# DhairyaLGandhi/FluxDistributed.jl

Measured on AMD Instinct MI355X. Metric: images/sec, higher is better.
Workload: dtype bf16; 1 GPU; model=resnet34, global_batch=96, image_size=224, num_classes=1000, parallelism=dp1, engine=graph, optimizer=sgd_momentum(lr=0.01,m=0.9), loss=logitcrossentropy

## Files before the change

fluxdistributed_amd/csrc/bindings.cpp:

```cpp
#include <torch/extension.h>
#include <ATen/hip/HIPContext.h>

#include "fda_kernels.h"

namespace {

using fda::DT;

DT dt_of(const at::Tensor& t) {
    if (t.scalar_type() == at::kBFloat16) return DT::BF16;
    TORCH_CHECK(t.scalar_type() == at::kFloat, "expected f32 or bf16, got ",
                t.scalar_type());
    return DT::F32;
}

hipStream_t cur_stream() {
    return at::hip::getCurrentHIPStream().stream();
}

std::pair<int64_t, int64_t> nhwc_rows(const at::Tensor& x) {
    TORCH_CHECK(x.dim() == 4, "expected 4D NCHW-logical tensor");
    TORCH_CHECK(x.is_contiguous(at::MemoryFormat::ChannelsLast),
                "expected channels_last layout");
    return {x.size(0) * x.size(2) * x.size(3), x.size(1)};
// ... 701 lines not shown
    TORCH_CHECK(w.size(1) == x.size(1), op, ": channel mismatch");
    return g;
}

at::Tensor conv_igemm_fwd(at::Tensor x, at::Tensor w,
                          int64_t sy, int64_t sx, int64_t py, int64_t px) {
    const char* op = "conv_igemm_fwd";
    const auto g = check_fwd(op, x, w, sy, sx, py, px);
    return std::get<0>(conv_run(op, fda::CONV_FWD, x, w, g, false, {}));
}

std::tuple<at::Tensor, at::Tensor> conv_igemm_fwd_stats(
    at::Tensor x, at::Tensor w, int64_t sy, int64_t sx, int64_t py,
    int64_t px) {
    const char* op = "conv_igemm_fwd_stats";
    const auto g = check_fwd(op, x, w, sy, sx, py, px);
    return conv_run(op, fda::CONV_FWD, x, w, g, true, {});
}

at::Tensor conv_igemm_dgrad(at::Tensor dy, at::Tensor wt,
                            int64_t C, int64_t H, int64_t W,
                            int64_t R, int64_t S,
                            int64_t sy, int64_t sx, int64_t py, int64_t px,
                            c10::optional<at::Tensor> accum) {
    const char* op = "conv_igemm_dgrad";
    check_cl_bf16(op, "dy", dy);
    const auto g = conv_geometry(op, dy.size(0), C, H, W, dy.size(1), R, S,
                                 sy, sx, py, px);
    check_dy(op, dy, g);
    TORCH_CHECK(wt.dim() == 2 && wt.scalar_type() == at::kBFloat16 &&
                    wt.is_contiguous() && wt.size(0) == R * S * C &&
                    wt.size(1) == g.K,
                op, ": wt must be contiguous bf16 [R*S*C][K]");
    ConvExtras ex;
    if (accum.has_value() && accum->defined()) {
        ex.accum = *accum;
        TORCH_CHECK(ex.accum.scalar_type() == at::kBFloat16 &&
                        ex.accum.sizes() == at::IntArrayRef({g.N, C, H, W}) &&
                        ex.accum.is_contiguous(at::MemoryFormat::ChannelsLast),
                    op, ": accum must be channels_last bf16 of dx's shape [",
                    g.N, ",", C, ",", H, ",", W, "]");
        check_aligned16(op, "accum", ex.accum);
    }
    return std::get<0>(conv_run(op, fda::CONV_DGRAD, dy, wt, g, false, ex));
}

fda::ConvGeom check_wgrad(const char* op, const at::Tensor& dy,
                          const at::Tensor& x, int64_t R, int64_t S,
                          int64_t sy, int64_t sx, int64_t py, int64_t px) {
    check_cl_bf16(op, "dy", dy);
    check_cl_bf16(op, "x", x);
    const auto g = conv_geometry(op, x.size(0), x.size(1), x.size(2),
                                 x.size(3), dy.size(1), R, S, sy, sx, py, px);
    TORCH_CHECK(dy.size(0) == x.size(0), op, ": batch size mismatch: dy has ",
                dy.size(0), ", x has ", x.size(0));
    check_dy(op, dy, g);
    return g;
}

void conv_igemm_wgrad_into(at::Tensor dy, at::Tensor x, at::Tensor ws,
                           int64_t R, int64_t S,
                           int64_t sy, int64_t sx, int64_t py, int64_t px) {
    const char* op = "conv_igemm_wgrad_into";
    const auto g = check_wgrad(op, dy, x, R, S, sy, sx, py, px);
    check_flat(op, "ws", ws, at::kFloat, (int64_t)g.K * R * S * g.C);
    check_device(op, {dy, x, ws});
    fda::conv_wgrad_launch(dy.data_ptr(), x.data_ptr(), ws.data_ptr<float>(),
                           g, cur_stream());
}

at::Tensor conv_igemm_wgrad(at::Tensor dy, at::Tensor x,
                            int64_t R, int64_t S,
                            int64_t sy, int64_t sx, int64_t py, int64_t px) {
    TORCH_CHECK(dy.dim() == 4 && x.dim() == 4,
                "conv_igemm_wgrad: dy and x must be 4-D");
    auto ws = at::zeros({dy.size(1), R * S * x.size(1)},
                        x.options().dtype(at::kFloat));
    conv_igemm_wgrad_into(dy, x, ws, R, S, sy, sx, py, px);
    return ws;
}

fda::ConvGeom check_stem_geometry(const char* op, const at::Tensor& x8,
                                  int64_t K, int64_t R, int64_t sy, int64_t sx,
                                  int64_t P, int64_t Q) {
    TORCH_CHECK(x8.scalar_type() == at::kBFloat16 && x8.dim() == 4 &&
                    x8.is_contiguous(at::MemoryFormat::ChannelsLast) &&
                    x8.size(1) == 8,
                op, ": x8 must be [N,8,Hp,Wp] channels_last bf16");
    TORCH_CHECK(K >= 64 && K % 64 == 0, op, ": K must be a multiple of 64");
    TORCH_CHECK(R >= 1 && sy >= 1 && sx >= 1 && P >= 1 && Q >= 1 &&
                    (P - 1) * sy + R <= x8.size(2) &&
                    (Q - 1) * sx + 8 <= x8.size(3),
                op, ": output ", P, "x", Q, " reads outside the padded ",
                x8.size(2), "x", x8.size(3), " input");
    fda::ConvGeom g{};
    g.N = (int)x8.size(0); g.H = (int)x8.size(2); g.W = (int)x8.size(3);
    g.C = 8; g.K = (int)K; g.P = (int)P; g.Q = (int)Q; g.R = (int)R; g.S = 1;
    g.sy = (int)sy; g.sx = (int)sx;
    return g;
}

std::tuple<at::Tensor, at::Tensor> conv_stem_run(
    const char* op, const at::Tensor& x8, const at::Tensor& wpad, int64_t R,
    int64_t sy, int64_t sx, int64_t P, int64_t Q, bool want_stats,
    const ConvExtras& ex) {
    TORCH_CHECK(wpad.dim() == 3 && wpad.is_contiguous() &&
                    wpad.scalar_type() == at::kBFloat16 &&
                    wpad.size(1) == R && wpad.size(2) == 64,
                op, ": wpad must be contiguous bf16 [K][R][64]");
    const auto g = check_stem_geometry(op, x8, wpad.size(0), R, sy, sx, P, Q);
    if (ex.scale.defined()) check_epilogue_coeffs(op, ex.scale, ex.shift, g.K);
    check_device(op, {x8, wpad, ex.scale, ex.shift});
    auto y = at::empty({g.N, g.K, g.P, g.Q},
                       x8.options().memory_format(at::MemoryFormat::ChannelsLast));
    at::Tensor part;
    if (want_stats)
        part = at::empty(
            {fda::conv_igemm_plan(g, fda::CONV_STEM).stats_rows, 2, g.K},
            x8.options().dtype(at::kFloat));
    const fda::EpiInfer epi{
        ex.scale.defined() ? ex.scale.data_ptr<float>() : nullptr,
        ex.scale.defined() ? ex.shift.data_ptr<float>() : nullptr, nullptr,
        ex.relu};
    fda::conv_stem_fwd_launch(x8.data_ptr(), wpad.data_ptr(), y.data_ptr(), g,
                              cur_stream(),
                              want_stats ? part.data_ptr<float>() : nullptr,
                              ex.scale.defined() ? &epi : nullptr);
    return {y, part};
}

at::Tensor conv_stem_fwd(at::Tensor x8, at::Tensor wpad, int64_t R,
                         int64_t sy, int64_t sx, int64_t P, int64_t Q) {
    return std::get<0>(conv_stem_run("conv_stem_fwd", x8, wpad, R, sy, sx, P,
                                     Q, false, {}));
}

std::tuple<at::Tensor, at::Tensor> conv_stem_fwd_stats(
    at::Tensor x8, at::Tensor wpad, int64_t R, int64_t sy, int64_t sx,
    int64_t P, int64_t Q) {
    return conv_stem_run("conv_stem_fwd_stats", x8, wpad, R, sy, sx, P, Q,
                         true, {});
}

std::tuple<int64_t, int64_t, int64_t, bool> conv_igemm_fwd_config(
    int64_t M, int64_t C, int64_t K, int64_t R, int64_t S) {
    TORCH_CHECK(M >= 1 && M <= INT32_MAX && C >= 64 && C % 64 == 0 &&
                    K >= 64 && K % 64 == 0 && R >= 1 && S >= 1,
                "conv_igemm_fwd_config: bad geometry");
    fda::ConvGeom g{};
    g.N = 1; g.P = 1; g.Q = (int)M;
    g.C = (int)C; g.K = (int)K; g.R = (int)R; g.S = (int)S;
    const auto plan = fda::conv_igemm_plan(g, fda::CONV_FWD);
    return {plan.bm, plan.bn, plan.sk, plan.ring};
}


at::Tensor conv_igemm_fwd_fused(at::Tensor x, at::Tensor w, at::Tensor scale,
                                at::Tensor shift, at::Tensor residual,
                                bool relu, int64_t sy, int64_t sx, int64_t py,
                                int64_t px) {
    const char* op = "conv_igemm_fwd_fused";
    const auto g = check_fwd(op, x, w, sy, sx, py, px);
    check_epilogue_coeffs(op, scale, shift, g.K);
    ConvExtras ex;
    ex.scale = scale;
    ex.shift = shift;
    ex.relu = relu;
    if (residual.defined() && residual.numel() > 0) {
        TORCH_CHECK(residual.scalar_type() == at::kBFloat16 &&
                        residual.sizes() ==
                            at::IntArrayRef({g.N, g.K, g.P, g.Q}) &&
                        residual.is_contiguous(at::MemoryFormat::ChannelsLast),
                    op, ": residual must be channels_last bf16 of the "
                    "output's shape [", g.N, ",", g.K, ",", g.P, ",", g.Q, "]");
        check_aligned16(op, "residual", residual);
        ex.residual = residual;
    }
    return std::get<0>(conv_run(op, fda::CONV_FWD, x, w, g, false, ex));
}

at::Tensor conv_stem_fwd_fused(at::Tensor x8, at::Tensor wpad,
                               at::Tensor scale, at::Tensor shift, bool relu,
                               int64_t R, int64_t sy, int64_t sx, int64_t P,
                               int64_t Q) {
    ConvExtras ex;
    ex.scale = scale;
    ex.shift = shift;
    ex.relu = relu;
    return std::get<0>(conv_stem_run("conv_stem_fwd_fused", x8, wpad, R, sy,
                                     sx, P, Q, false, ex));
}

void bn_fold_eval_batch(at::Tensor w_ptrs, at::Tensor b_ptrs,
                        at::Tensor rm_ptrs, at::Tensor rv_ptrs, at::Tensor Cs,
                        at::Tensor offs, at::Tensor eps, at::Tensor arena,
                        int64_t max_c) {
    const char* op = "bn_fold_eval_batch";
    const int64_t n = w_ptrs.numel();
    TORCH_CHECK(n >= 1 && n <= 65535, op, ": need 1..65535 layers, got ", n);
    check_flat(op, "w_ptrs", w_ptrs, at::kLong, n);
    check_flat(op, "b_ptrs", b_ptrs, at::kLong, n);
    check_flat(op, "rm_ptrs", rm_ptrs, at::kLong, n);
    check_flat(op, "rv_ptrs", rv_ptrs, at::kLong, n);
    check_flat(op, "Cs", Cs, at::kInt, n);
    check_flat(op, "offs", offs, at::kLong, n);
    check_flat(op, "eps", eps, at::kFloat, n);
    TORCH_CHECK(arena.scalar_type() == at::kFloat && arena.dim() == 1 &&
                    arena.is_contiguous(),
                op, ": arena must be 1-D contiguous fp32");
    TORCH_CHECK(max_c >= 1 && 2 * max_c <= arena.numel(), op,
                ": max_c must be in [1, arena/2], got ", max_c);
    check_device(op, {w_ptrs, b_ptrs, rm_ptrs, rv_ptrs, Cs, offs, eps, arena});
    fda::bn_fold_eval_batch_launch(
        w_ptrs.data_ptr<int64_t>(), b_ptrs.data_ptr<int64_t>(),
        rm_ptrs.data_ptr<int64_t>(), rv_ptrs.data_ptr<int64_t>(),
        Cs.data_ptr<int>(), offs.data_ptr<int64_t>(), eps.data_ptr<float>(),
        arena.data_ptr<float>(), arena.numel(), (int)n, (int)max_c,
        cur_stream());
}

at::Tensor conv_stem_wgrad(at::Tensor dy, at::Tensor x8, int64_t R,
                           int64_t sy, int64_t sx) {
    const char* op = "conv_stem_wgrad";
    TORCH_CHECK(dy.scalar_type() == at::kBFloat16 && dy.dim() == 4 &&
                    dy.is_contiguous(at::MemoryFormat::ChannelsLast),
                op, ": dy must be 4-D channels_last bf16");
    const auto g = check_stem_geometry(op, x8, dy.size(1), R, sy, sx,
                                       dy.size(2), dy.size(3));
    TORCH_CHECK(dy.size(0) == x8.size(0), op, ": batch size mismatch");
    check_device(op, {dy, x8});
    auto ws = at::zeros({g.K, R * 64}, x8.options().dtype(at::kFloat));
    fda::conv_stem_wgrad_launch(dy.data_ptr(), x8.data_ptr(),
                                ws.data_ptr<float>(), g, cur_stream());
    return ws;
}

at::Tensor pad_rows_bf16(at::Tensor src, int64_t ldl) {
    TORCH_CHECK(src.dim() == 2 && src.is_contiguous() &&
                src.scalar_type() == at::kBFloat16);
    const long M = src.size(0);
    const int C = (int)src.size(1);
    TORCH_CHECK(C % 8 == 0 && ldl % 8 == 0 && ldl >= C);
    check_device("pad_rows_bf16", {src});
    auto dst = at::empty({M, ldl}, src.options());
    fda::pad_rows_bf16_launch(dst.data_ptr(), src.data_ptr(), M, C, (int)ldl,
                              cur_stream());
    return dst;
}

void pad_rows_bf16_into(at::Tensor dst, at::Tensor src) {
    TORCH_CHECK(dst.dim() == 2 && src.dim() == 2);
    TORCH_CHECK(dst.is_contiguous() && src.is_contiguous());
    TORCH_CHECK(dst.size(0) == src.size(0));
    TORCH_CHECK(dst.scalar_type() == at::kBFloat16 &&
                    src.scalar_type() == at::kBFloat16,
                "pad_rows_bf16_into: bf16 only");
    TORCH_CHECK(src.size(1) % 8 == 0 && dst.size(1) % 8 == 0 &&
                    src.size(1) <= dst.size(1),
                "pad_rows_bf16_into: row lengths must be multiples of 8 "
                "with src's <= dst's");
    check_device("pad_rows_bf16_into", {dst, src});
    fda::pad_rows_bf16_launch(dst.data_ptr(), src.data_ptr(), src.size(0),
                              (int)src.size(1), (int)dst.size(1),
                              cur_stream());
}

void bias_add_rows_bf16(at::Tensor y, at::Tensor bias) {
    TORCH_CHECK(y.dim() == 2 && y.is_contiguous() &&
                y.scalar_type() == at::kBFloat16);
    TORCH_CHECK(bias.numel() == y.size(1) && bias.is_contiguous() &&
                bias.scalar_type() == at::kBFloat16);
    TORCH_CHECK(y.size(1) % 8 == 0, "bias_add_rows_bf16: row length % 8");
    check_device("bias_add_rows_bf16", {y, bias});
    fda::bias_add_rows_bf16_launch(y.data_ptr(), bias.data_ptr(), y.size(0),
                                   (int)y.size(1), cur_stream());
}

void colsum_accum_bf16(at::Tensor g, at::Tensor dy) {
    TORCH_CHECK(dy.dim() == 2 && dy.is_contiguous() &&
                dy.scalar_type() == at::kBFloat16);
    TORCH_CHECK(g.is_contiguous() && g.scalar_type() == at::kBFloat16);
    TORCH_CHECK(g.numel() <= dy.size(1));
    check_device("colsum_accum_bf16", {g, dy});
    fda::colsum_accum_bf16_launch(g.data_ptr(), dy.data_ptr(), dy.size(0),
                                  (int)dy.size(1), (int)g.numel(),
                                  cur_stream());
}

void grad_accum_batch(at::Tensor g_ptrs, at::Tensor ws_ptrs, at::Tensor ns,
                      int64_t max_n) {
    const int64_t n = g_ptrs.numel();
    check_flat("grad_accum_batch", "g_ptrs", g_ptrs, at::kLong, n);
    check_flat("grad_accum_batch", "ws_ptrs", ws_ptrs, at::kLong, n);
    check_flat("grad_accum_batch", "ns", ns, at::kLong, n);
    check_device("grad_accum_batch", {g_ptrs, ws_ptrs, ns});
    fda::grad_accum_batch_launch(g_ptrs.data_ptr<int64_t>(),
                                 ws_ptrs.data_ptr<int64_t>(),
                                 ns.data_ptr<int64_t>(),
                                 (int)g_ptrs.numel(), max_n, cur_stream());
}

void grad_accum_bf16(at::Tensor g, at::Tensor ws) {
    TORCH_CHECK(g.scalar_type() == at::kBFloat16 && g.is_contiguous());
    TORCH_CHECK(ws.scalar_type() == at::kFloat && ws.is_contiguous());
    TORCH_CHECK(g.numel() == ws.numel());
    check_device("grad_accum_bf16", {g, ws});
// ... 47 lines not shown

at::Tensor preprocess_batch(at::Tensor arena, at::Tensor meta, int64_t crop,
                            bool normalize, bool standardize, bool bf16) {
    TORCH_CHECK(arena.is_cuda() && meta.is_cuda(),
                "preprocess_batch: device tensors required (a CPU tensor here "
                "would fault the GPU with a host pointer)");
    TORCH_CHECK(arena.device() == meta.device(),
                "preprocess_batch: arena and meta must share a device");
    TORCH_CHECK(arena.scalar_type() == at::kByte && arena.dim() == 1 &&
                arena.is_contiguous(),
                "preprocess_batch: arena must be 1-D contiguous uint8");
    TORCH_CHECK(meta.scalar_type() == at::kInt && meta.dim() == 2 &&
                meta.size(1) == fda::PREPROCESS_META_INTS &&
                meta.is_contiguous(),
                "preprocess_batch: meta must be contiguous int32 [N][",
                fda::PREPROCESS_META_INTS, "]");
    TORCH_CHECK((reinterpret_cast<uintptr_t>(arena.data_ptr()) & 15) == 0,
                "preprocess_batch: arena must be 16-byte aligned");
    TORCH_CHECK(crop >= 1 && crop <= 4096,
                "preprocess_batch: crop must be in [1, 4096], got ", crop);
    const int64_t N = meta.size(0);
    const int tiles = fda::preprocess_tiles((int)crop);
    TORCH_CHECK(N * tiles < (int64_t)1 << 31,
                "preprocess_batch: batch too large");
    auto out = at::empty({N, 3, crop, crop},
                         arena.options()
                             .dtype(bf16 ? at::kBFloat16 : at::kFloat)
                             .memory_format(at::MemoryFormat::ChannelsLast));
    if (N == 0) return out;
    auto scratch = at::empty({N, crop, crop, 3},
                             arena.options().dtype(at::kFloat));
    auto partials = at::empty({N, tiles, 2},
                              arena.options().dtype(at::kDouble));
    auto stream = cur_stream();
    fda::preprocess_resample_launch(arena.data_ptr<uint8_t>(), arena.numel(),
                                    meta.data_ptr<int32_t>(),
                                    scratch.data_ptr<float>(),
                                    partials.data_ptr<double>(), (int)N,
                                    (int)crop, normalize, stream);
    fda::preprocess_apply_launch(scratch.data_ptr<float>(),
                                 partials.data_ptr<double>(), out.data_ptr(),
                                 (int)N, (int)crop, standardize,
                                 bf16 ? DT::BF16 : DT::F32, stream);
    return out;
}

}

PYBIND11_MODULE(TORCH_EXTENSION_NAME, m) {
    m.def("preprocess_batch", &preprocess_batch, pybind11::arg("arena"),
          pybind11::arg("meta"), pybind11::arg("crop"),
          pybind11::arg("normalize"), pybind11::arg("standardize"),
          pybind11::arg("bf16"),
          "uint8 image arena -> resized, cropped, normalized NHWC batch");
    m.def("ce_fwd", &ce_fwd, "fused logit cross-entropy fwd (loss + dlogits)");
    m.def("add_relu_fwd", &add_relu_fwd);
    m.def("add_relu_bwd", &add_relu_bwd);
    m.def("bn_act_fwd", &bn_act_fwd, pybind11::arg("x"),
          pybind11::arg("weight"), pybind11::arg("bias"),
          pybind11::arg("running_mean"), pybind11::arg("running_var"),
          pybind11::arg("training"), pybind11::arg("momentum"),
          pybind11::arg("eps"), pybind11::arg("relu"),
          pybind11::arg("residual"),
          pybind11::arg("conv_part") = pybind11::none());
    m.def("bn_act_bwd", &bn_act_bwd, pybind11::arg("gout"),
          pybind11::arg("x"), pybind11::arg("weight"),
          pybind11::arg("save_mean"), pybind11::arg("save_invstd"),
          pybind11::arg("out"), pybind11::arg("relu"),
          pybind11::arg("training"),
          pybind11::arg("gw_out") = pybind11::none(),
          pybind11::arg("gb_out") = pybind11::none(),
          pybind11::arg("want_gres") = false,
          pybind11::arg("bias") = pybind11::none());
    m.def("bn_act_pool_supported", &bn_act_pool_supported);
    m.def("bn_act_pool_fwd", &bn_act_pool_fwd, pybind11::arg("x"),
          pybind11::arg("weight"), pybind11::arg("bias"),
          pybind11::arg("running_mean"), pybind11::arg("running_var"),
          pybind11::arg("training"), pybind11::arg("momentum"),
          pybind11::arg("eps"), pybind11::arg("KH"), pybind11::arg("KW"),
          pybind11::arg("S"), pybind11::arg("P"),
          pybind11::arg("conv_part") = pybind11::none());
    m.def("bn_act_pool_bwd", &bn_act_pool_bwd, pybind11::arg("gout"),
          pybind11::arg("x"), pybind11::arg("weight"), pybind11::arg("bias"),
          pybind11::arg("save_mean"), pybind11::arg("save_invstd"),
          pybind11::arg("idx"), pybind11::arg("KH"), pybind11::arg("KW"),
          pybind11::arg("S"), pybind11::arg("P"), pybind11::arg("training"),
          pybind11::arg("gw_out") = pybind11::none(),
          pybind11::arg("gb_out") = pybind11::none());
    m.def("maxpool_fwd", &maxpool_fwd);
    m.def("maxpool_bwd", &maxpool_bwd);
    m.def("gap_fwd", &gap_fwd);
    m.def("gap_bwd", &gap_bwd);
    m.def("sgd_step", &sgd_step);
    m.def("adam_step", &adam_step);
    m.def("lars_plan", &lars_plan, pybind11::arg("offsets"),
          pybind11::arg("numels"), pybind11::arg("n"),
          pybind11::arg("seg_base"),
          "host chunk table of one flat group: int32 [nchunks][3] rows of "
          "{segment id, start element, own elements}");
    m.def("lars_norms", &lars_norms, pybind11::arg("P"), pybind11::arg("G"),
          pybind11::arg("M"), pybind11::arg("table"),
          pybind11::arg("partials"), pybind11::arg("chunk_base"),
          pybind11::arg("total_chunks"), pybind11::arg("S"));
    m.def("lars_fold", &lars_fold, pybind11::arg("partials"),
          pybind11::arg("seg_meta"), pybind11::arg("lr"),
          pybind11::arg("coef"), pybind11::arg("stats"),
          pybind11::arg("skipped"), pybind11::arg("eta"),
          pybind11::arg("weight_decay"), pybind11::arg("eps"),
          pybind11::arg("max_grad_norm"));
    m.def("lars_step", &lars_step, pybind11::arg("P"), pybind11::arg("G"),
          pybind11::arg("M"), pybind11::arg("V"), pybind11::arg("table"),
          pybind11::arg("seg_meta"), pybind11::arg("coef"),
          pybind11::arg("stats"), pybind11::arg("momentum"),
          pybind11::arg("weight_decay"));
    m.attr("LARS_CHUNK") = fda::LARS_CHUNK;
    m.def("grad_mean_multi", &grad_mean_multi, pybind11::arg("grads"),
          pybind11::arg("flag") = pybind11::none(),
          "in-place mean of R flat gradient buffers (fp32 sum, one round)");
    m.def("conv_igemm_fwd_stats", &conv_igemm_fwd_stats);
    m.def("conv_stem_fwd_stats", &conv_stem_fwd_stats);
    m.def("conv_igemm_fwd", &conv_igemm_fwd,
          "implicit-GEMM conv fwd (NHWC bf16, MFMA)");
    m.def("wt_transpose_batch", &wt_transpose_batch);
    m.def("grad_accum_bf16", &grad_accum_bf16);
    m.def("grad_accum_batch", &grad_accum_batch);
    m.def("pad_rows_bf16", &pad_rows_bf16);
    m.def("pad_rows_bf16_into", &pad_rows_bf16_into);
    m.def("bias_add_rows_bf16", &bias_add_rows_bf16);
    m.def("colsum_accum_bf16", &colsum_accum_bf16);
    m.def("conv_stem_fwd", &conv_stem_fwd);
    m.def("conv_stem_wgrad", &conv_stem_wgrad);
    m.def("conv_igemm_fwd_config", &conv_igemm_fwd_config,
          pybind11::arg("M"), pybind11::arg("C"), pybind11::arg("K"),
          pybind11::arg("R"), pybind11::arg("S"),
          "(BM, BN, SK, ring) of a forward conv with M output pixels");
    m.def("conv_igemm_fwd_fused", &conv_igemm_fwd_fused, pybind11::arg("x"),
          pybind11::arg("w"), pybind11::arg("scale"), pybind11::arg("shift"),
          pybind11::arg("residual"), pybind11::arg("relu"),
          pybind11::arg("sy"), pybind11::arg("sx"), pybind11::arg("py"),
          pybind11::arg("px"),
          "conv + eval BN + residual + ReLU, one bf16 round (inference)");
    m.def("conv_stem_fwd_fused", &conv_stem_fwd_fused, pybind11::arg("x8"),
          pybind11::arg("wpad"), pybind11::arg("scale"),
          pybind11::arg("shift"), pybind11::arg("relu"), pybind11::arg("R"),
          pybind11::arg("sy"), pybind11::arg("sx"), pybind11::arg("P"),
          pybind11::arg("Q"));
    m.def("bn_fold_eval_batch", &bn_fold_eval_batch, pybind11::arg("w_ptrs"),
          pybind11::arg("b_ptrs"), pybind11::arg("rm_ptrs"),
          pybind11::arg("rv_ptrs"), pybind11::arg("Cs"),
          pybind11::arg("offs"), pybind11::arg("eps"), pybind11::arg("arena"),
          pybind11::arg("max_c"),
          "eval-mode BN scale/shift of every layer in one launch");
    m.def("conv_igemm_wgrad_into", &conv_igemm_wgrad_into);
    m.def("conv_igemm_wgrad", &conv_igemm_wgrad,
          "implicit-GEMM conv weight-grad (NHWC bf16, MFMA + tr16 reads)");
    m.def("conv_igemm_dgrad", &conv_igemm_dgrad,
          "implicit-GEMM conv input-grad (NHWC bf16, MFMA; optional fused "
          "+= accum epilogue)",
          pybind11::arg("dy"), pybind11::arg("wt"), pybind11::arg("C"),
          pybind11::arg("H"), pybind11::arg("W"), pybind11::arg("R"),
          pybind11::arg("S"), pybind11::arg("sy"), pybind11::arg("sx"),
          pybind11::arg("py"), pybind11::arg("px"),
          pybind11::arg("accum") = pybind11::none());
    m.attr("_built_for") = "gfx950";
}
```

fluxdistributed_amd/csrc/conv_igemm.hip:

```cpp

#include <hip/hip_runtime.h>
#include <cassert>
#include <cstdlib>
#include "fda_common.h"
#include "fda_kernels.h"

namespace fda {

typedef __attribute__((ext_vector_type(8))) short short8;
typedef __attribute__((ext_vector_type(4))) float floatx4;

__device__ __align__(16) static const unsigned short conv_zero16[8] = {0};

#define FDA_GLDS16(gptr, lptr)                                              \
    __builtin_amdgcn_global_load_lds(                                       \
        (const __attribute__((address_space(1))) void*)(gptr),              \
        (__attribute__((address_space(3))) void*)(lptr), 16, 0, 0)


constexpr int BK = 64;

template <class E>
__device__ __forceinline__ const E& epi_of(const E& e) { return e; }

// ... 552 lines not shown
        hipLaunchKernelGGL(conv_skcombine_kernel<EpiInfer>, grid, dim3(256),
                           0, stream, part, (unsigned short*)y,
                           (float*)nullptr, M, OC, SK,
                           (const unsigned short*)nullptr, *epi);
    else
        hipLaunchKernelGGL(conv_skcombine_kernel<>, grid, dim3(256), 0,
                           stream, part, (unsigned short*)y, stats, M, OC, SK,
                           (const unsigned short*)accsrc);
}

void conv_stem_fwd_launch(const void* src, const void* wgt, void* out,
                          const ConvGeom& g, hipStream_t stream, float* stats,
                          const EpiInfer* epi) {
    if (epi != nullptr)
        launch_cfg<CONV_STEM, 256, 64, 1, 2, BK, EpiInfer>(
            src, wgt, out, g, 1, stream, nullptr, nullptr, nullptr, *epi);
    else
        launch_cfg<CONV_STEM, 256, 64, 1>(src, wgt, out, g, 1, stream, stats,
                                          nullptr, nullptr);
}

static bool conv_bk32() {
    static const bool v = [] {
        const char* e = getenv("FLUXDIST_CONV_BK32");
        return e ? atoi(e) != 0 : true;
    }();
    return v;
}

ConvPlan conv_igemm_plan(const ConvGeom& g, ConvMode mode) {
    const int OC = g.oc(mode);
    const long M = g.rows(mode);
    ConvPlan p;
    const bool big = OC % 128 == 0 && mode != CONV_STEM;
    p.bm = big ? 128 : 256;
    p.bn = big ? 128 : 64;
    const long mtiles = (M + p.bm - 1) / p.bm;
    const long blocks1 = mtiles * (OC / p.bn) * g.classes(mode);
    p.sk = 1;
    if (mode != CONV_STEM && g.classes(mode) == 1 && g.depth(mode) >= 48) {
        if (blocks1 < 192) p.sk = 4;
        else if (blocks1 < 384) p.sk = 2;
    }
    p.blocks = blocks1 * p.sk;
    p.ring = mode != CONV_STEM && conv_bk32() &&
             p.blocks >= (p.bn == 128 ? 576 : 512);
    p.stats_rows = mode == CONV_DGRAD ? 0
                 : p.sk > 1 ? conv_skcombine_blocks(M, OC) : mtiles;
    return p;
}

template <int MODE, class... EPI>
static void conv_dispatch(const void* src, const void* wgt, void* out,
                          const ConvGeom& g, const ConvPlan& p,
                          hipStream_t stream, float* stats, float* skpart,
                          const void* accsrc, EPI... epi) {
    if (p.bn == 128) {
        if (p.ring)
            launch_cfg<MODE, 128, 128, 2, 3, 32, EPI...>(
                src, wgt, out, g, p.sk, stream, stats, skpart, accsrc, epi...);
        else
            launch_cfg<MODE, 128, 128, 2, 2, BK, EPI...>(
                src, wgt, out, g, p.sk, stream, stats, skpart, accsrc, epi...);
    } else {
        if (p.ring)
            launch_cfg<MODE, 256, 64, 1, 3, 32, EPI...>(
                src, wgt, out, g, p.sk, stream, stats, skpart, accsrc, epi...);
        else
            launch_cfg<MODE, 256, 64, 1, 2, BK, EPI...>(
                src, wgt, out, g, p.sk, stream, stats, skpart, accsrc, epi...);
    }
}

void conv_igemm_launch(const void* src, const void* wgt, void* out,
                       const ConvGeom& g, ConvMode mode, const ConvPlan& plan,
                       hipStream_t stream, float* stats, float* skpart,
                       const void* accsrc, const EpiInfer* epi) {
    assert(epi == nullptr || (mode == CONV_FWD && stats == nullptr &&
                              accsrc == nullptr));
    if (mode == CONV_DGRAD)
        conv_dispatch<CONV_DGRAD>(src, wgt, out, g, plan, stream, stats,
                                  skpart, accsrc);
    else if (epi != nullptr && plan.sk == 1)
        conv_dispatch<CONV_FWD, EpiInfer>(src, wgt, out, g, plan, stream,
                                          nullptr, nullptr, nullptr, *epi);
    else
        conv_dispatch<CONV_FWD>(src, wgt, out, g, plan, stream, stats, skpart,
                                accsrc);
}

__global__ __launch_bounds__(256) void wt_transpose_kernel(
    const long* __restrict__ src_ptrs,
    long* __restrict__ dst_ptrs,
    const int* __restrict__ Ks, const int* __restrict__ RCs,
    const int* __restrict__ tile_counts) {
    const int t = blockIdx.y;
    const int K = Ks[t], RC = RCs[t];
    const int kt = K / 64, rt = RC / 64;
    if ((int)blockIdx.x >= tile_counts[t]) return;
    const int tk = blockIdx.x % kt, trc = blockIdx.x / kt;
    (void)rt;
    const unsigned short* src = (const unsigned short*)src_ptrs[t];
    unsigned short* dst = (unsigned short*)dst_ptrs[t];

    __shared__ unsigned short tile[64][64 + 8];
    const int tid = threadIdx.x;
    #pragma unroll
    for (int i = 0; i < 2; ++i) {
        const int kk = (tid / 8) + i * 32;
        const int rc = (tid % 8) * 8;
        const unsigned short* sp =
            src + (long)(tk * 64 + kk) * RC + trc * 64 + rc;
        #pragma unroll
        for (int e = 0; e < 8; ++e) tile[kk][rc + e] = sp[e];
    }
    __syncthreads();
    #pragma unroll
    for (int i = 0; i < 2; ++i) {
        const int rc = (tid / 8) + i * 32;
        const int kk = (tid % 8) * 8;
        unsigned short* dp =
            dst + (long)(trc * 64 + rc) * K + tk * 64 + kk;
        #pragma unroll
        for (int e = 0; e < 8; ++e) dp[e] = tile[kk + e][rc];
    }
}

void wt_transpose_launch(const long* src_ptrs, long* dst_ptrs, const int* Ks,
                         const int* RCs, const int* tile_counts, int ntensors,
                         int max_tiles, hipStream_t stream) {
    dim3 grid((unsigned)max_tiles, (unsigned)ntensors);
    hipLaunchKernelGGL(wt_transpose_kernel, grid, dim3(256), 0, stream,
                       src_ptrs, dst_ptrs, Ks, RCs, tile_counts);
}

typedef __attribute__((ext_vector_type(4))) short short4_;

constexpr int WG_BM = 64;
constexpr int WG_MCH = 2048;

template <int FT, bool STEM = false>
__global__ __launch_bounds__(256, 2) void conv_wgrad_kernel(
    const unsigned short* __restrict__ dy,
    const unsigned short* __restrict__ x,
    float* __restrict__ ws,
    int N, int H, int W, int C, int K, int P, int Q,
    int R, int S, int sy, int sx, int py, int px, int nch, int mch) {
    constexpr int MB = WG_BM;
    constexpr int TCH = 32 * FT;
    constexpr int TILE_ELEMS = MB * TCH;
    constexpr int GI = MB * TCH / 2048;
    constexpr int NWIN = MB / 4;
    constexpr int KSN = MB / 32;
    const int rs = blockIdx.z / nch;
    const int chunk = blockIdx.z % nch;
    const int r = rs / S, s = rs % S;
    const int k0 = blockIdx.x * TCH;
    const int c0 = blockIdx.y * TCH;
    const long M = (long)N * P * Q;
    const long mb0 = (long)chunk * mch;
    const long mend = (mb0 + mch < M) ? mb0 + mch : M;

    const int tid = threadIdx.x;
    const int lane = tid & 63;
    const int wid = tid >> 6;
    const int wk = wid >> 1;
    const int wc = wid & 1;

    extern __shared__ unsigned short lds[];

    const floatx4 zero4 = {0.f, 0.f, 0.f, 0.f};
    floatx4 acc[FT][FT];
    #pragma unroll
    for (int ki = 0; ki < FT; ++ki)
        #pragma unroll
        for (int ci = 0; ci < FT; ++ci) acc[ki][ci] = zero4;

    int st_q[GI], st_p[GI], st_n[GI], st_ch[GI];
    long st_dyoff[GI];
    long st_m[GI];
    #pragma unroll
    for (int i = 0; i < GI; ++i) {
        const int ln = (wid * GI + i) * 64 + lane;
        const int e8 = ln * 8;
        const int kb = e8 / (MB * 16);
        const int rr = e8 % (MB * 16);
        const int pos = rr >> 6;
        const int v = (pos < NWIN / 2) ? pos * 2
                                       : (pos - NWIN / 2) * 2 + 1;
        const int ml = (v << 2) + ((rr & 63) >> 4);
        const int ch = (kb << 4) + (rr & 15);
        st_ch[i] = ch;
        const long m = mb0 + ml;
        st_m[i] = m;
        st_q[i] = (int)(m % Q);
        st_p[i] = (int)((m / Q) % P);
        st_n[i] = (int)(m / ((long)Q * P));
        st_dyoff[i] = m * K + k0 + ch;
    }
    const int dQ = MB % Q, dP = (MB / Q) % P, dN0 = MB / (Q * P);
    const long dDY = (long)MB * K;

    auto stage = [&](int buf) {
        unsigned short* base = lds + buf * 2 * TILE_ELEMS;
        #pragma unroll
        for (int i = 0; i < GI; ++i) {
            const unsigned short* sp =
                (st_m[i] < mend) ? dy + st_dyoff[i] : conv_zero16;
            FDA_GLDS16(sp, base + (wid * GI + i) * 512);
        }
        #pragma unroll
        for (int i = 0; i < GI; ++i) {
            const unsigned short* sp = conv_zero16;
            if (st_m[i] < mend) {
                if (STEM) {
                    const int hh = st_p[i] * sy + r;
                    const int ww = st_q[i] * sx;
                    sp = x + (((long)st_n[i] * H + hh) * W + ww) * 8 +
                         st_ch[i];
                } else {
                    const int hh = st_p[i] * sy - py + r;
                    const int ww = st_q[i] * sx - px + s;
                    if ((unsigned)hh < (unsigned)H && (unsigned)ww < (unsigned)W)
                        sp = x + (((long)st_n[i] * H + hh) * W + ww) * C +
                             c0 + st_ch[i];
                }
            }
            FDA_GLDS16(sp, base + TILE_ELEMS + (wid * GI + i) * 512);
        }
        #pragma unroll
        for (int i = 0; i < GI; ++i) {
            st_m[i] += MB;
            st_dyoff[i] += dDY;
            int q = st_q[i] + dQ;
            int p = st_p[i] + dP;
            int n = st_n[i] + dN0;
            if (q >= Q) { q -= Q; ++p; }
            if (p >= P) { p -= P; ++n; }
            if (p >= P) { p -= P; ++n; }
            st_q[i] = q; st_p[i] = p; st_n[i] = n;
        }
    };

    const int l15 = lane & 15, lg = lane >> 4;

    constexpr int RING = (FT == 2) ? 3 : 2;
    const int nsteps = (int)((mend - mb0 + MB - 1) / MB);
    if (nsteps > 0) stage(0);
    if (RING > 2 && nsteps > 1) stage(1);
    for (int it = 0; it < nsteps; ++it) {
        if (RING > 2 && it + 1 < nsteps) {
            static_assert(2 * GI == 4 || 2 * GI == 8,
                          "counted ring: state the vmcnt for this GI");
            if constexpr (2 * GI == 4)
                asm volatile("s_waitcnt vmcnt(4)" ::: "memory");
            else
                asm volatile("s_waitcnt vmcnt(8)" ::: "memory");
        } else {
            asm volatile("s_waitcnt vmcnt(0)" ::: "memory");
        }
        __builtin_amdgcn_s_barrier();
        const unsigned short* buf = lds + (it % RING) * 2 * TILE_ELEMS;
        short4_ a[FT][KSN][2], b[FT][KSN][2];
        #pragma unroll
        for (int fi = 0; fi < FT; ++fi)
            #pragma unroll
            for (int ks = 0; ks < KSN; ++ks) {
                const int kb_a = wk * FT + fi;
                const int kb_b = wc * FT + fi;
                const int v0 = ks * 8 + lg * 2;
                const int p0 = (v0 >> 1);
                const int p1 = p0 + NWIN / 2;
                const unsigned short* pa =
                    buf + kb_a * (MB * 16) + l15 * 4;
                const unsigned short* pb =
                    buf + TILE_ELEMS + kb_b * (MB * 16) + l15 * 4;
                a[fi][ks][0] = __builtin_amdgcn_ds_read_tr16_b64_v4i16(
                    (__attribute__((address_space(3))) short4_*)(pa + p0 * 64));
                a[fi][ks][1] = __builtin_amdgcn_ds_read_tr16_b64_v4i16(
                    (__attribute__((address_space(3))) short4_*)(pa + p1 * 64));
                b[fi][ks][0] = __builtin_amdgcn_ds_read_tr16_b64_v4i16(
                    (__attribute__((address_space(3))) short4_*)(pb + p0 * 64));
                b[fi][ks][1] = __builtin_amdgcn_ds_read_tr16_b64_v4i16(
                    (__attribute__((address_space(3))) short4_*)(pb + p1 * 64));
            }
        if (it + RING - 1 < nsteps) stage((it + RING - 1) % RING);
        __builtin_amdgcn_s_setprio(1);
        #pragma unroll
        for (int ks = 0; ks < KSN; ++ks)
            #pragma unroll
            for (int ki = 0; ki < FT; ++ki)
                #pragma unroll
                for (int ci = 0; ci < FT; ++ci) {
                    short8 af, bf;
                    #pragma unroll
                    for (int e = 0; e < 4; ++e) {
                        af[e] = a[ki][ks][0][e];
                        af[e + 4] = a[ki][ks][1][e];
                        bf[e] = b[ci][ks][0][e];
                        bf[e + 4] = b[ci][ks][1][e];
                    }
                    acc[ki][ci] = __builtin_amdgcn_mfma_f32_16x16x32_bf16(
                        af, bf, acc[ki][ci], 0, 0, 0);
                }
        __builtin_amdgcn_s_setprio(0);
    }

    const int fcol = lane & 15, frow0 = (lane >> 4) * 4;
    const long RSC = (long)R * S * C;
    #pragma unroll
    for (int ki = 0; ki < FT; ++ki)
        #pragma unroll
        for (int ci = 0; ci < FT; ++ci)
            #pragma unroll
            for (int jj = 0; jj < 4; ++jj) {
                const int kk = k0 + wk * 16 * FT + ki * 16 + frow0 + jj;
                const int cc = c0 + wc * 16 * FT + ci * 16 + fcol;
                atomicAdd(&ws[kk * RSC + (long)rs * C + cc],
                          acc[ki][ci][jj]);
            }
}

void conv_stem_wgrad_launch(const void* dy, const void* x, float* ws,
                            const ConvGeom& g, hipStream_t stream) {
    const long M = g.rows(CONV_STEM);
    constexpr int STEM_MCH = 8 * WG_MCH;
    const int nch = (int)((M + STEM_MCH - 1) / STEM_MCH);
    dim3 grid((unsigned)(g.K / 64), 1u, (unsigned)(g.R * nch));
    const size_t shmem = 3 * 2 * (WG_BM * 64) * sizeof(unsigned short);
    hipLaunchKernelGGL((conv_wgrad_kernel<2, true>), grid, dim3(256), shmem,
                       stream, (const unsigned short*)dy,
                       (const unsigned short*)x, ws, g.N, g.H, g.W, 64, g.K,
                       g.P, g.Q, g.R, 1, g.sy, g.sx, 0, 0, nch, STEM_MCH);
}

static int pick_mch(long M, long tiles, int target) {
    long nch_t = target / (tiles > 0 ? tiles : 1);
    if (nch_t < 1) nch_t = 1;
    long mch = (M + nch_t - 1) / nch_t;
    mch = ((mch + WG_MCH - 1) / WG_MCH) * WG_MCH;
    if (mch < WG_MCH) mch = WG_MCH;
    return (int)mch;
}

static void conv_wgrad_plan(long M, int C, int K, int R, int S,
                            int* ft, int* mch, int* nch) {
    const long tiles4 = (long)(K / 128) * (C / 128) * R * S;
    const long blocks4_max = tiles4 * ((M + WG_MCH - 1) / WG_MCH);
    if (K % 128 == 0 && C % 128 == 0 && blocks4_max >= 192) {
        *ft = 4;
        *mch = pick_mch(M, tiles4, 768);
    } else {
        *ft = 2;
        *mch = pick_mch(M, (long)(K / 64) * (C / 64) * R * S, 768);
    }
    *nch = (int)((M + *mch - 1) / *mch);
}

void conv_wgrad_launch(const void* dy, const void* x, float* ws,
                       const ConvGeom& g, hipStream_t stream) {
    int FTp, mch, nch;
    conv_wgrad_plan(g.rows(CONV_FWD), g.C, g.K, g.R, g.S, &FTp, &mch, &nch);
    auto launch = [&](auto kern, int tch, size_t shmem) {
        dim3 grid((unsigned)(g.K / tch), (unsigned)(g.C / tch),
                  (unsigned)(g.R * g.S * nch));
        hipLaunchKernelGGL(kern, grid, dim3(256), shmem, stream,
                           (const unsigned short*)dy,
                           (const unsigned short*)x, ws, g.N, g.H, g.W, g.C,
                           g.K, g.P, g.Q, g.R, g.S, g.sy, g.sx, g.py, g.px,
                           nch, mch);
    };
    if (FTp == 4)
        launch(conv_wgrad_kernel<4>, 128,
               2 * 2 * (WG_BM * 128) * sizeof(unsigned short));
    else
        launch(conv_wgrad_kernel<2>, 64,
               3 * 2 * (WG_BM * 64) * sizeof(unsigned short));
}

}
```

fluxdistributed_amd/csrc/fda_common.h:

```cpp
#pragma once
#include <hip/hip_runtime.h>
#include <hip/hip_bf16.h>
#include <cstdint>

namespace fda {

constexpr int WAVE = 64;

__device__ __forceinline__ float to_f32(float v) { return v; }
__device__ __forceinline__ float to_f32(__hip_bfloat16 v) { return __bfloat162float(v); }
__device__ __forceinline__ float bf16bits_to_f32(unsigned short u) {
    union { unsigned int i; float f; } c;
    c.i = (unsigned int)u << 16;
    return c.f;
}
__device__ __forceinline__ unsigned short f32_to_bf16bits(float f) {
    union { float f; unsigned int i; } c;
    c.f = f;
    unsigned int x = c.i;
    unsigned int lsb = (x >> 16) & 1u;
    x += 0x7fffu + lsb;
    return (unsigned short)(x >> 16);
}

template <typename T> struct VecWidth;
template <> struct VecWidth<float> { static constexpr int value = 4; };
template <> struct VecWidth<unsigned short> { static constexpr int value = 8; };

template <typename T>
__device__ __forceinline__ float load_f32(const T* p) {
    if constexpr (sizeof(T) == 2) return bf16bits_to_f32(*(const unsigned short*)p);
    else return *(const float*)p;
}
template <typename T>
__device__ __forceinline__ void store_f32(T* p, float v) {
    if constexpr (sizeof(T) == 2) *(unsigned short*)p = f32_to_bf16bits(v);
    else *(float*)p = v;
}

template <typename T, int V>
__device__ __forceinline__ void unpack_f32(const uint4& raw, float (&f)[V]) {
    const unsigned w[4] = {raw.x, raw.y, raw.z, raw.w};
    if constexpr (sizeof(T) == 2) {
        static_assert(V == 8, "16 B of bf16");
        #pragma unroll
        for (int i = 0; i < 4; ++i) {
            f[2 * i] = __uint_as_float(w[i] << 16);
            f[2 * i + 1] = __uint_as_float(w[i] & 0xffff0000u);
        }
    } else {
        static_assert(V == 4, "16 B of fp32");
        #pragma unroll
        for (int i = 0; i < 4; ++i) f[i] = __uint_as_float(w[i]);
    }
}

__device__ __forceinline__ float bn_scale_of(float weight, float invstd) {
    return __fmul_rn(weight, invstd);
}
__device__ __forceinline__ float bn_shift_of(float bias, float mean,
                                             float scale) {
    return __fmaf_rn(-mean, scale, bias);
}
__device__ __forceinline__ float bn_affine(float x, float scale, float shift) {
    return __fmaf_rn(x, scale, shift);
}
__device__ __forceinline__ float bn_bwd_dx(float g, float xhat, float k1,
                                           float k2, float weight,
                                           float invstd) {
    return (g - k1 - xhat * k2) * weight * invstd;
}
template <typename T, int V>
__device__ __forceinline__ void round_storage(float (&f)[V]) {
    if constexpr (sizeof(T) == 2) {
        #pragma unroll
        for (int i = 0; i < V; ++i) {
            T t;
            store_f32(&t, f[i]);
            f[i] = load_f32(&t);
        }
    }
}

template <typename T>
__device__ __forceinline__ bool bn_relu_positive(float x, float scale,
                                                 float shift) {
    T t;
    store_f32(&t, fmaxf(bn_affine(x, scale, shift), 0.f));
    return load_f32(&t) > 0.f;
}

__device__ __forceinline__ unsigned xcd_contiguous_block(unsigned bid,
                                                         unsigned nwg) {
    const unsigned q = nwg / 8, r = nwg % 8, xcd = bid % 8;
    const unsigned base = xcd < r ? xcd * (q + 1) : r * (q + 1) + (xcd - r) * q;
    return base + bid / 8;
}

__device__ __forceinline__ float wave_reduce_sum(float v) {
    #pragma unroll
    for (int off = WAVE / 2; off > 0; off >>= 1) v += __shfl_down(v, off, WAVE);
    return v;
}
__device__ __forceinline__ float wave_reduce_max(float v) {
    #pragma unroll
    for (int off = WAVE / 2; off > 0; off >>= 1) v = fmaxf(v, __shfl_down(v, off, WAVE));
    return v;
}

__device__ __forceinline__ float block_reduce_sum(float v, float* scratch) {
    const int lane = threadIdx.x & (WAVE - 1);
    const int wid = threadIdx.x / WAVE;
    const int nw = blockDim.x / WAVE;
    v = wave_reduce_sum(v);
    if (lane == 0) scratch[wid] = v;
    __syncthreads();
    float r = (lane < nw) ? scratch[lane] : 0.f;
    r = wave_reduce_sum(r);
    r = __shfl(r, 0, WAVE);
    __syncthreads();
    if (threadIdx.x == 0) scratch[0] = r;
    __syncthreads();
    return scratch[0];
}
__device__ __forceinline__ float block_reduce_max(float v, float* scratch) {
    const int lane = threadIdx.x & (WAVE - 1);
    const int wid = threadIdx.x / WAVE;
    const int nw = blockDim.x / WAVE;
    v = wave_reduce_max(v);
    if (lane == 0) scratch[wid] = v;
    __syncthreads();
    float r = (lane < nw) ? scratch[lane] : -INFINITY;
    r = wave_reduce_max(r);
    r = __shfl(r, 0, WAVE);
    __syncthreads();
    if (threadIdx.x == 0) scratch[0] = r;
    __syncthreads();
    return scratch[0];
}

template <int V> struct ChanAcc { float v[V]; };

template <int V>
__device__ __forceinline__ void block_fold_rows(ChanAcc<V> s, ChanAcc<V> q,
                                                float* smem, float* out,
                                                int tpr, int stride) {
    const int rpb = blockDim.x / tpr;
    const int lane_c = threadIdx.x % tpr;
    const int sub_r = threadIdx.x / tpr;
    #pragma unroll
    for (int pass = 0; pass < 2; ++pass) {
        const float* loc = pass == 0 ? s.v : q.v;
        #pragma unroll
        for (int k = 0; k < V; ++k) smem[threadIdx.x * V + k] = loc[k];
        __syncthreads();
        if (sub_r == 0) {
            float acc[V];
            #pragma unroll
            for (int k = 0; k < V; ++k) acc[k] = 0.f;
            for (int rr = 0; rr < rpb; ++rr) {
                const float* src = smem + (rr * tpr + lane_c) * V;
                #pragma unroll
                for (int k = 0; k < V; ++k) acc[k] += src[k];
            }
            #pragma unroll
            for (int k = 0; k < V; ++k)
                out[pass * stride + lane_c * V + k] = acc[k];
        }
        __syncthreads();
    }
}

}
```

fluxdistributed_amd/csrc/fda_kernels.h:

```cpp
#pragma once
#include <hip/hip_runtime.h>
#include <cstdint>
#include <type_traits>

namespace fda {

enum class DT { F32 = 0, BF16 = 1 };

template <typename F>
inline void dispatch_dtype(DT dt, F&& f) {
    if (dt == DT::BF16) f((unsigned short)0, std::integral_constant<int, 8>{});
    else f(0.f, std::integral_constant<int, 4>{});
}
template <typename F>
inline void dispatch_flag(bool flag, F&& f) {
    if (flag) f(std::true_type{});
    else f(std::false_type{});
}

inline int grid_1d(int64_t n, int cap) {
    const int64_t b = (n + 255) / 256;
    return (int)(b < 1 ? 1 : (b > cap ? cap : b));
}

void ce_fwd_launch(const void* logits, const int64_t* target, float* loss,
                   void* dlogits, int N, int C, int ldl, DT dt,
                   hipStream_t s);

void add_relu_fwd_launch(const void* x, const void* r, void* out, int64_t n,
                         DT dt, hipStream_t s);
void add_relu_bwd_launch(const void* gout, const void* out, void* gx, int64_t n,
                         DT dt, hipStream_t s);

int bn_stats_partial_floats(int C, int64_t rows, DT dt);
void bn_stats_launch(const void* x, float* ws, float* part,
                     const float* weight, const float* bias,
                     float* running_mean, float* running_var, float* save_mean,
                     float* save_invstd, int64_t rows, int C, float momentum,
                     float eps, DT dt, hipStream_t s);
void bn_partial_prefold_launch(const float* part, float* out, int NB,
                               int NB2, int chunkC, hipStream_t s);
void bn_fwd_finalize_launch(const float* part, int NB, int chunkC, int c_base,
                            const float* weight, const float* bias, float* rm,
                            float* rv, float* save_mean, float* save_invstd,
                            float* ws, int64_t rows, int C, float momentum,
                            float eps, hipStream_t s);

void bn_eval_finalize_launch(float* ws, const float* weight,
                             const float* bias, const float* running_mean,
                             const float* running_var, float* save_mean,
                             float* save_invstd, int C, float eps,
                             hipStream_t s);
void bn_apply_launch(const void* x, const void* residual, void* out,
                     const float* ws , int64_t rows, int C,
                     bool relu, DT dt, hipStream_t s);
void bn_fold_eval_batch_launch(const long* w_ptrs, const long* b_ptrs,
                               const long* rm_ptrs, const long* rv_ptrs,
                               const int* Cs, const long* offs,
                               const float* eps, float* arena, long arena_len,
                               int nlayers, int max_c, hipStream_t s);

void bn_bwd_stats_launch(const void* gout, const void* x, const void* out,
                         const float* save_mean, const float* save_invstd,
                         float* ws, float* part, float* gw, float* gb,
                         int64_t rows, int C, bool relu, bool training,
                         bool accum_g, DT dt, hipStream_t s,
                         const float* weight = nullptr,
                         const float* bias = nullptr);
void bn_bwd_apply_launch(const void* gout, const void* x, const void* out,
                         const float* save_mean, const float* save_invstd,
                         const float* weight, const float* ws, void* gx,
                         void* gres, int64_t rows, int C, bool relu, DT dt,
                         hipStream_t s, const float* bias = nullptr);
void bn_bwd_finalize_launch(const float* part, int NB, int chunkC, int c_base,
                            float* ws, float* gw, float* gb, int64_t rows,
                            int C, bool training, bool accum_g, hipStream_t s);

void maxpool_fwd_launch(const void* x, void* out, uint8_t* idx, int N, int H,
                        int W, int C, int HO, int WO, int KH, int KW, int S,
                        int P, DT dt, hipStream_t s);
void maxpool_bwd_launch(const void* gout, const uint8_t* idx, void* gx, int N,
                        int H, int W, int C, int HO, int WO, int KH, int KW,
                        int S, int P, DT dt, hipStream_t s);

void bn_relu_maxpool_fwd_launch(const void* x, const float* ws, void* out,
                                uint8_t* idx, int N, int H, int W, int C,
                                int HO, int WO, int KH, int KW, int S, int P,
                                DT dt, hipStream_t s);
int bn_relu_maxpool_bwd_blocks(int N, int H);
void bn_relu_maxpool_bwd_stats_launch(
    const void* gout, const uint8_t* idx, const void* x,
    const float* save_mean, const float* save_invstd, const float* weight,
    const float* bias, float* part, int N, int H, int W, int C, int HO,
    int WO, int KH, int KW, int S, int P, DT dt, hipStream_t s);
void bn_relu_maxpool_bwd_apply_launch(
    const void* gout, const uint8_t* idx, const void* x,
    const float* save_mean, const float* save_invstd, const float* weight,
    const float* bias, const float* ws, void* gx, int N, int H, int W, int C,
    int HO, int WO, int KH, int KW, int S, int P, DT dt, hipStream_t s);

void gap_fwd_launch(const void* x, void* y, int N, int HW, int C, DT dt,
                    hipStream_t s);
void gap_bwd_launch(const void* gy, void* gx, int N, int HW, int C, DT dt,
                    hipStream_t s);

enum ConvMode { CONV_FWD = 0, CONV_DGRAD = 1, CONV_STEM = 2 };

struct ConvGeom {
    int N, H, W, C, K, P, Q, R, S, sy, sx, py, px;
    int oc(ConvMode m) const { return m == CONV_DGRAD ? C : K; }
    int classes(ConvMode m) const { return m == CONV_DGRAD ? sy * sx : 1; }
    long rows(ConvMode m) const {
        return m == CONV_DGRAD
            ? (long)N * ((H + sy - 1) / sy) * ((W + sx - 1) / sx)
            : (long)N * P * Q;
    }
    long depth(ConvMode m) const {
        return m == CONV_STEM ? R : (long)R * S * ((m == CONV_DGRAD ? K : C) / 64);
    }
};

struct ConvPlan {
    int bm, bn, sk;
    bool ring;
    long blocks;
    long stats_rows;
};
ConvPlan conv_igemm_plan(const ConvGeom& g, ConvMode mode);

struct EpiInfer {
    const float* scale;
    const float* shift;
    const unsigned short* residual;
    int relu;
};

void conv_igemm_launch(const void* src, const void* wgt, void* out,
                       const ConvGeom& g, ConvMode mode, const ConvPlan& plan,
                       hipStream_t stream, float* stats = nullptr,
                       float* skpart = nullptr, const void* accsrc = nullptr,
                       const EpiInfer* epi = nullptr);

void conv_skcombine_launch(const float* part, void* y, float* stats, long M,
                           int OC, int SK, hipStream_t stream,
                           const void* accsrc = nullptr,
                           const EpiInfer* epi = nullptr);

void conv_stem_fwd_launch(const void* src, const void* wgt, void* out,
                          const ConvGeom& g, hipStream_t stream,
                          float* stats = nullptr,
                          const EpiInfer* epi = nullptr);
void conv_stem_wgrad_launch(const void* dy, const void* x, float* ws,
                            const ConvGeom& g, hipStream_t stream);

void conv_wgrad_launch(const void* dy, const void* x, float* ws,
                       const ConvGeom& g, hipStream_t stream);

void wt_transpose_launch(const long* src_ptrs, long* dst_ptrs, const int* Ks,
                         const int* RCs, const int* tile_counts, int ntensors,
                         int max_tiles, hipStream_t stream);

void grad_accum_bf16_launch(void* g, const float* ws, long n, hipStream_t s);
void grad_accum_batch_launch(const long* g_ptrs, const long* ws_ptrs,
                             const long* ns, int ntensors, long max_n,
                             hipStream_t s);

void pad_rows_bf16_launch(void* dst, const void* src, long M, int C, int ldl,
                          hipStream_t s);
void bias_add_rows_bf16_launch(void* y, const void* bias, long M, int ldl,
                               hipStream_t s);
void colsum_accum_bf16_launch(void* g, const void* dy, long M, int ldl,
                              int Cvalid, hipStream_t s);

constexpr int PREPROCESS_META_INTS = 10;
int preprocess_tiles(int crop);
void preprocess_resample_launch(const uint8_t* arena, int64_t arena_bytes,
                                const int32_t* meta, float* scratch,
                                double* partials, int N, int crop,
                                bool normalize, hipStream_t s);
void preprocess_apply_launch(const float* scratch, const double* partials,
                             void* out, int N, int crop, bool standardize,
                             DT dt, hipStream_t s);

void sgd_step_launch(void* P, const void* G, float* M, float* V, int64_t n,
                     float lr, float mom, float wd, bool nesterov,
                     bool has_master, DT dt, hipStream_t s);
void adam_step_launch(void* P, const void* G, float* M, float* V, float* S,
                      int64_t n, float lr, float b1, float b2, float eps,
                      float wd, float bc1, float bc2, bool has_master, DT dt,
                      hipStream_t s);

constexpr int LARS_CHUNK = 4096;
constexpr int LARS_ROW_INTS = 3;
constexpr int LARS_SEG_INTS = 3;
constexpr int LARS_STATS_HEAD = 2;
void lars_norms_launch(const void* P, const void* G, const float* M,
                       const int32_t* table, int nchunks, double* partials,
                       int64_t n, int S, bool has_master, DT dt,
                       hipStream_t s);
void lars_fold_launch(const double* partials, int total_chunks,
                      const int32_t* seg_meta, int S, const float* lr,
                      float eta, float wd, float eps, float max_grad_norm,
                      float* coef, float* stats, int* skipped, hipStream_t s);
void lars_step_launch(void* P, const void* G, float* M, float* V,
                      const int32_t* table, int nchunks,
                      const int32_t* seg_meta, const float* coef,
                      const float* stats, int64_t n, int S, float mom,
                      float wd, bool has_master, DT dt, hipStream_t s);

constexpr int GRAD_MEAN_MAX_R = 16;
void grad_mean_multi_launch(void* const* bufs, int R, int64_t n,
                            int* nonfinite, DT dt, hipStream_t s);

}
```

Before: 12250 images/sec.

## Flatten wgrad grid with XCD-contiguous block mapping and occupancy-based split-M plan

The weight-gradient conv kernel now runs on a 1D grid. Each block id is remapped so that consecutive logical tiles land on the same XCD, then decoded into (ktile, ctile, rs, chunk), with the same M chunk of neighbouring k/c tiles kept together for L2 reuse. The split-M planner now sizes chunks from a CU-slot target (256 CUs times blocks per CU, halved for 1x1 convs) with a smaller minimum chunk, in place of a fixed 768-block target rounded to 2048 rows. This changes the balance between parallelism and atomicAdd traffic into the fp32 workspace. Host-side bindings that expose the plan and coordinate mapping are added for testing.

Result: faster. 12860 images/sec, median of 6 (+5.0%).

```diff
diff --git a/fluxdistributed_amd/csrc/bindings.cpp b/fluxdistributed_amd/csrc/bindings.cpp
--- a/fluxdistributed_amd/csrc/bindings.cpp
+++ b/fluxdistributed_amd/csrc/bindings.cpp
@@ -877,6 +877,28 @@
     g.C = (int)C; g.K = (int)K; g.R = (int)R; g.S = (int)S;
     const auto plan = fda::conv_igemm_plan(g, fda::CONV_FWD);
     return {plan.bm, plan.bn, plan.sk, plan.ring};
+}
+
+std::tuple<int64_t, int64_t, int64_t, int64_t> conv_igemm_wgrad_config(
+    int64_t M, int64_t C, int64_t K, int64_t R, int64_t S) {
+    TORCH_CHECK(M >= 1 && M <= INT32_MAX && C >= 64 && C % 64 == 0 &&
+                    K >= 64 && K % 64 == 0 && R >= 1 && S >= 1,
+                "conv_igemm_wgrad_config: bad geometry");
+    const auto p = fda::conv_wgrad_plan(M, (int)C, (int)K, (int)R, (int)S);
+    return {p.ft, p.mch, p.nch, p.nwg};
+}
+
+std::tuple<int64_t, int64_t, int64_t, int64_t> conv_wgrad_block_coords(
+    int64_t bid, int64_t ktiles, int64_t ctiles, int64_t RS, int64_t nch) {
+    TORCH_CHECK(ktiles >= 1 && ctiles >= 1 && RS >= 1 && nch >= 1 &&
+                    ktiles * ctiles * RS * nch <= INT32_MAX,
+                "conv_wgrad_block_coords: bad grid");
+    TORCH_CHECK(bid >= 0 && bid < ktiles * ctiles * RS * nch,
+                "conv_wgrad_block_coords: bid ", bid, " outside the grid of ",
+                ktiles * ctiles * RS * nch, " blocks");
+    const auto c = fda::wgrad_block_coords((unsigned)bid, (int)ktiles,
+                                           (int)ctiles, (int)RS, (int)nch);
+    return {c.ktile, c.ctile, c.rs, c.chunk};
 }
 
 
@@ -1230,6 +1252,10 @@
           pybind11::arg("max_c"),
           "eval-mode BN scale/shift of every layer in one launch");
     m.def("conv_igemm_wgrad_into", &conv_igemm_wgrad_into);
+    m.def("conv_igemm_wgrad_config", &conv_igemm_wgrad_config,
+          "The (FT, mch, nch, nwg) plan a body wgrad with M pixels runs");
+    m.def("conv_wgrad_block_coords", &conv_wgrad_block_coords,
+          "Block id -> (ktile, ctile, rs, chunk) of a wgrad grid");
     m.def("conv_igemm_wgrad", &conv_igemm_wgrad,
           "implicit-GEMM conv weight-grad (NHWC bf16, MFMA + tr16 reads)");
     m.def("conv_igemm_dgrad", &conv_igemm_dgrad,
diff --git a/fluxdistributed_amd/csrc/conv_igemm.hip b/fluxdistributed_amd/csrc/conv_igemm.hip
--- a/fluxdistributed_amd/csrc/conv_igemm.hip
+++ b/fluxdistributed_amd/csrc/conv_igemm.hip
@@ -728,11 +728,13 @@
     constexpr int GI = MB * TCH / 2048;
     constexpr int NWIN = MB / 4;
     constexpr int KSN = MB / 32;
-    const int rs = blockIdx.z / nch;
-    const int chunk = blockIdx.z % nch;
+    const WgradCoords bc = wgrad_block_coords(blockIdx.x, K / TCH, C / TCH,
+                                              R * S, nch);
+    const int rs = bc.rs;
+    const int chunk = bc.chunk;
     const int r = rs / S, s = rs % S;
-    const int k0 = blockIdx.x * TCH;
-    const int c0 = blockIdx.y * TCH;
+    const int k0 = bc.ktile * TCH;
+    const int c0 = bc.ctile * TCH;
     const long M = (long)N * P * Q;
     const long mb0 = (long)chunk * mch;
     const long mend = (mb0 + mch < M) ? mb0 + mch : M;
@@ -902,7 +904,7 @@
     const long M = g.rows(CONV_STEM);
     constexpr int STEM_MCH = 8 * WG_MCH;
     const int nch = (int)((M + STEM_MCH - 1) / STEM_MCH);
-    dim3 grid((unsigned)(g.K / 64), 1u, (unsigned)(g.R * nch));
+    const dim3 grid((unsigned)((g.K / 64) * g.R * nch));
     const size_t shmem = 3 * 2 * (WG_BM * 64) * sizeof(unsigned short);
     hipLaunchKernelGGL((conv_wgrad_kernel<2, true>), grid, dim3(256), shmem,
                        stream, (const unsigned short*)dy,
@@ -910,47 +912,43 @@
                        g.P, g.Q, g.R, 1, g.sy, g.sx, 0, 0, nch, STEM_MCH);
 }
 
-static int pick_mch(long M, long tiles, int target) {
-    long nch_t = target / (tiles > 0 ? tiles : 1);
-    if (nch_t < 1) nch_t = 1;
-    long mch = (M + nch_t - 1) / nch_t;
-    mch = ((mch + WG_MCH - 1) / WG_MCH) * WG_MCH;
-    if (mch < WG_MCH) mch = WG_MCH;
-    return (int)mch;
-}
-
-static void conv_wgrad_plan(long M, int C, int K, int R, int S,
-                            int* ft, int* mch, int* nch) {
+constexpr int WG_CUS = 256;
+constexpr int WG_MIN_MCH = 7 * WG_BM;
+
+WgradPlan conv_wgrad_plan(long M, int C, int K, int R, int S) {
+    WgradPlan p;
     const long tiles4 = (long)(K / 128) * (C / 128) * R * S;
+    const long tiles2 = (long)(K / 64) * (C / 64) * R * S;
     const long blocks4_max = tiles4 * ((M + WG_MCH - 1) / WG_MCH);
-    if (K % 128 == 0 && C % 128 == 0 && blocks4_max >= 192) {
-        *ft = 4;
-        *mch = pick_mch(M, tiles4, 768);
-    } else {
-        *ft = 2;
-        *mch = pick_mch(M, (long)(K / 64) * (C / 64) * R * S, 768);
-    }
-    *nch = (int)((M + *mch - 1) / *mch);
+    p.ft = (K % 128 == 0 && C % 128 == 0 && blocks4_max >= 192) ? 4 : 2;
+    const long tiles = p.ft == 4 ? tiles4 : tiles2;
+    const long slots = WG_CUS * (p.ft == 4 ? 2 : 3);
+    long nch = (R * S == 1 ? slots / 2 : slots) / tiles;
+    if (nch < 1) nch = 1;
+    long mch = ((M + nch - 1) / nch + WG_BM - 1) / WG_BM * WG_BM;
+    if (mch < WG_MIN_MCH) mch = WG_MIN_MCH;
+    if (M <= 2 * WG_MCH) mch = WG_MCH;
+    p.mch = (int)mch;
+    p.nch = (int)((M + mch - 1) / mch);
+    p.nwg = tiles * p.nch;
+    return p;
 }
 
 void conv_wgrad_launch(const void* dy, const void* x, float* ws,
                        const ConvGeom& g, hipStream_t stream) {
-    int FTp, mch, nch;
-    conv_wgrad_plan(g.rows(CONV_FWD), g.C, g.K, g.R, g.S, &FTp, &mch, &nch);
-    auto launch = [&](auto kern, int tch, size_t shmem) {
-        dim3 grid((unsigned)(g.K / tch), (unsigned)(g.C / tch),
-                  (unsigned)(g.R * g.S * nch));
-        hipLaunchKernelGGL(kern, grid, dim3(256), shmem, stream,
-                           (const unsigned short*)dy,
+    const WgradPlan p = conv_wgrad_plan(g.rows(CONV_FWD), g.C, g.K, g.R, g.S);
+    auto launch = [&](auto kern, size_t shmem) {
+        hipLaunchKernelGGL(kern, dim3((unsigned)p.nwg), dim3(256), shmem,
+                           stream, (const unsigned short*)dy,
                            (const unsigned short*)x, ws, g.N, g.H, g.W, g.C,
                            g.K, g.P, g.Q, g.R, g.S, g.sy, g.sx, g.py, g.px,
-                           nch, mch);
+                           p.nch, p.mch);
     };
-    if (FTp == 4)
-        launch(conv_wgrad_kernel<4>, 128,
+    if (p.ft == 4)
+        launch(conv_wgrad_kernel<4>,
                2 * 2 * (WG_BM * 128) * sizeof(unsigned short));
     else
-        launch(conv_wgrad_kernel<2>, 64,
+        launch(conv_wgrad_kernel<2>,
                3 * 2 * (WG_BM * 64) * sizeof(unsigned short));
 }
 
diff --git a/fluxdistributed_amd/csrc/fda_common.h b/fluxdistributed_amd/csrc/fda_common.h
--- a/fluxdistributed_amd/csrc/fda_common.h
+++ b/fluxdistributed_amd/csrc/fda_common.h
@@ -90,12 +90,6 @@
     return load_f32(&t) > 0.f;
 }
 
-__device__ __forceinline__ unsigned xcd_contiguous_block(unsigned bid,
-                                                         unsigned nwg) {
-    const unsigned q = nwg / 8, r = nwg % 8, xcd = bid % 8;
-    const unsigned base = xcd < r ? xcd * (q + 1) : r * (q + 1) + (xcd - r) * q;
-    return base + bid / 8;
-}
 
 __device__ __forceinline__ float wave_reduce_sum(float v) {
     #pragma unroll
diff --git a/fluxdistributed_amd/csrc/fda_kernels.h b/fluxdistributed_amd/csrc/fda_kernels.h
--- a/fluxdistributed_amd/csrc/fda_kernels.h
+++ b/fluxdistributed_amd/csrc/fda_kernels.h
@@ -152,6 +152,34 @@
                           const EpiInfer* epi = nullptr);
 void conv_stem_wgrad_launch(const void* dy, const void* x, float* ws,
                             const ConvGeom& g, hipStream_t stream);
+
+__host__ __device__ __forceinline__ unsigned xcd_contiguous_block(
+    unsigned bid, unsigned nwg) {
+    const unsigned q = nwg / 8, r = nwg % 8, xcd = bid % 8;
+    const unsigned base = xcd < r ? xcd * (q + 1) : r * (q + 1) + (xcd - r) * q;
+    return base + bid / 8;
+}
+
+struct WgradPlan {
+    int ft, mch, nch;
+    long nwg;
+};
+WgradPlan conv_wgrad_plan(long M, int C, int K, int R, int S);
+
+struct WgradCoords {
+    int ktile, ctile, rs, chunk;
+};
+__host__ __device__ __forceinline__ WgradCoords wgrad_block_coords(
+    unsigned bid, int ktiles, int ctiles, int RS, int nch) {
+    const unsigned nwg = (unsigned)(ktiles * ctiles * RS * nch);
+    unsigned L = xcd_contiguous_block(bid, nwg);
+    WgradCoords c;
+    c.ktile = (int)(L % (unsigned)ktiles); L /= (unsigned)ktiles;
+    c.ctile = (int)(L % (unsigned)ctiles); L /= (unsigned)ctiles;
+    c.rs = (int)(L % (unsigned)RS);
+    c.chunk = (int)(L / (unsigned)RS);
+    return c;
+}
 
 void conv_wgrad_launch(const void* dy, const void* x, float* ws,
                        const ConvGeom& g, hipStream_t stream);
```
